# rostin79s/TFHE-AES

Measured on AMD Instinct MI355X. Metric: AES-128 CTR blocks/sec (FHE), higher is better.
Workload: dtype u64+f64; 1 GPU; configs[2]: 128 CTR blocks per GPU, Server::aes_encrypt 10 rounds (1280 bit-CBS/block), counters pre-incremented client-side; params=PARAM_OPT, blocks_per_gpu=128, total_blocks=128

## Files before the change

### tfhe_aes_amd/csrc/aes_schedule.h

```cpp
#pragma once

static int many_sbox_dev(fheaes_ctx *c, const uint64_t *bytes, uint64_t n_bytes, int set, uint64_t *out)
{
    return wopbs_dev(c, bytes, n_bytes, 8, c->lutset_d[set], (uint32_t)c->lutset_n[set], 0, out);
}

static int aes_rounds(uint32_t key_bits) { return key_bits == 128 ? 10 : key_bits == 192 ? 12 : key_bits == 256 ? 14 : 0; }

static int check_key_bits(fheaes_ctx *c, uint32_t key_bits)
{
    if (!aes_rounds(key_bits)) return c->fail(FHEAES_ERR_INVALID, "key_bits must be 128, 192 or 256, got %u", key_bits);
    return FHEAES_OK;
}

struct AesStep { int set; uint32_t n_luts; GatherTable table; int key_round; };
struct AesSchedule {
    int first_key_round = 0;
    uint32_t max_luts = 0;
    std::vector<AesStep> steps;
    void add(int set, uint32_t n_luts, const GatherTable &t, int key_round) { steps.push_back({set, n_luts, t, key_round}); max_luts = std::max(max_luts, n_luts); }
};

static AesSchedule aes_encrypt_schedule(int nr)
{
    AesSchedule s;
    s.first_key_round = 0;
    for (int round = 1; round < nr; ++round) s.add(LUTSET_ENC_ROUND, 3, table_enc_round(), round);
    s.add(LUTSET_SBOX, 1, table_shift_rows(false), nr);
    return s;
}

static AesSchedule aes_decrypt_schedule(int nr)
{
    AesSchedule s;
    s.first_key_round = nr;
    for (int round = nr; round >= 2; --round) {
        s.add(LUTSET_INV_SBOX, 1, table_shift_rows(true), round - 1);
        s.add(LUTSET_DEC_MUL, 4, table_dec_mix(), -1);
    }
    s.add(LUTSET_INV_SBOX, 1, table_shift_rows(true), 0);
    return s;
}

static AesSchedule aes_decrypt_eq_schedule(int nr)
{
    AesSchedule s;
    s.first_key_round = nr;
    for (int round = nr - 1; round >= 1; --round) s.add(LUTSET_DEC_EQ_ROUND, 4, table_dec_eq_round(), round);
    s.add(LUTSET_INV_SBOX, 1, table_shift_rows(true), 0);
    return s;
}

static int aes_run_dev(fheaes_ctx *c, const KeySets &rk, uint64_t *state, uint64_t n_blocks, const AesSchedule &sch)
{
    const uint64_t bw = 8ull * c->big1, sw = 16 * bw, steps = sch.steps.size();
    auto key_of = [&](const AesStep &st, uint64_t first_block) {
        if (st.key_round < 0) return KeySets{nullptr, nullptr, 0};
        return rk.round((uint64_t)st.key_round, sw, first_block);
    };
    const uint64_t w = aes_context_window(c, n_blocks, steps);
    TRY(ensure(c, c->ws_vp, (w ? w : n_blocks) * 16 * sch.max_luts * bw * 8));
    uint64_t *vp = (uint64_t *)c->ws_vp.p;
    TRY(launch_add_bcast(c, state, rk.round((uint64_t)sch.first_key_round, sw), sw, n_blocks));
    if (w == 0) {
        for (const AesStep &st : sch.steps) {
            TRY(many_sbox_dev(c, state, 16 * n_blocks, st.set, vp));
            TRY(launch_gather(c, vp, st.n_luts, key_of(st, 0), state, n_blocks, st.table));
        }
        return FHEAES_OK;
    }
    const uint64_t ggsw_words = (uint64_t)c->k1 * c->k1 * FHE_N, total = steps * n_blocks;
    TRY(ensure_wopbs_ws(c, w * AES_BLOCK_BITS));
    uint64_t *small = (uint64_t *)c->ws_small.p;
    const double2 *ggswf = (const double2 *)c->ws_ggswf.p;
    struct Segment { const AesStep *st; uint64_t first, blocks, row; uint64_t *vp; };
    for (uint64_t i0 = 0; i0 < total; i0 += w) {
        const uint64_t len = std::min<uint64_t>(w, total - i0), s = i0 / n_blocks, b0 = i0 % n_blocks, m = len * AES_BLOCK_BITS;
        Segment seg[2] = {{&sch.steps[s], b0, std::min<uint64_t>(len, n_blocks - b0), 0, vp}, {}};
        int n_seg = 1;
        if (seg[0].blocks < len) {
            seg[1] = {&sch.steps[s + 1], 0, len - seg[0].blocks, seg[0].blocks, vp + seg[0].blocks * 16 * seg[0].st->n_luts * bw};
            n_seg = 2;
        }
        for (int g = 0; g < n_seg; ++g)
            TRY(launch_keyswitch(c, state + seg[g].first * sw, seg[g].blocks * AES_BLOCK_BITS, small + seg[g].row * AES_BLOCK_BITS * (c->n + 1)));
        TRY(cbs_from_small(c, m));
        if (n_seg == 1 || seg[0].st->set == seg[1].st->set) {
            const int set = seg[0].st->set;
            TRY(launch_vertical_packing(c, ggswf, 16 * len, 8, c->lutset_d[set], (uint32_t)c->lutset_n[set], 0, vp));
        } else {
            for (int g = 0; g < n_seg; ++g) {
                const int set = seg[g].st->set;
                TRY(launch_vertical_packing(c, ggswf + seg[g].row * AES_BLOCK_BITS * (ggsw_words / 2), 16 * seg[g].blocks, 8, c->lutset_d[set],
                                            (uint32_t)c->lutset_n[set], 0, seg[g].vp));
            }
        }
        for (int g = 0; g < n_seg; ++g)
            TRY(launch_gather(c, seg[g].vp, seg[g].st->n_luts, key_of(*seg[g].st, seg[g].first), state + seg[g].first * sw, seg[g].blocks, seg[g].st->table));
    }
    return FHEAES_OK;
}

static int aes_encrypt_dev(fheaes_ctx *c, const KeySets &rk, uint64_t *state, uint64_t n_blocks, int nr) { return aes_run_dev(c, rk, state, n_blocks, aes_encrypt_schedule(nr)); }
static int aes_decrypt_dev(fheaes_ctx *c, const KeySets &rk, uint64_t *state, uint64_t n_blocks, int nr) { return aes_run_dev(c, rk, state, n_blocks, aes_decrypt_schedule(nr)); }
static int aes_decrypt_eq_dev(fheaes_ctx *c, const KeySets &dw, uint64_t *state, uint64_t n_blocks, int nr) { return aes_run_dev(c, dw, state, n_blocks, aes_decrypt_eq_schedule(nr)); }

typedef int (*AesDevFn)(fheaes_ctx *, const KeySets &, uint64_t *, uint64_t, int);

static int dec_round_keys_dev(fheaes_ctx *c, const uint64_t *w, uint64_t *dw, int nr, uint64_t n_keys)
{
    const uint64_t bw = 8ull * c->big1, sw = 16 * bw, ks = (uint64_t)(nr + 1) * sw, mid = (uint64_t)(nr - 1) * 16, nbytes = mid * n_keys;
    const bool strided = n_keys > 1;
    TRY(ensure(c, c->ws_vp, nbytes * 4 * bw * 8));
    TRY(ensure(c, c->ws_tmp_a, nbytes * bw * 8));
    if (strided) TRY(ensure(c, c->ws_tmp_b, nbytes * bw * 8));
    uint64_t *vp = (uint64_t *)c->ws_vp.p, *mix = (uint64_t *)c->ws_tmp_a.p, *flat = (uint64_t *)c->ws_tmp_b.p;
    TRY(launch_key_rows(c, dw, ks, w, ks, 0, nullptr, 0, 0, 16, n_keys, 1));
    TRY(launch_key_rows(c, dw + (uint64_t)nr * sw, ks, w + (uint64_t)nr * sw, ks, 0, nullptr, 0, 0, 16, n_keys, 1));
    if (strided) TRY(launch_key_rows(c, flat, mid * bw, w + sw, ks, 0, nullptr, 0, 0, (uint32_t)mid, n_keys, 1));
    TRY(many_sbox_dev(c, strided ? flat : w + sw, nbytes, LUTSET_DEC_MUL, vp));
    TRY(launch_gather(c, vp, 4, KeySets{nullptr, nullptr, 0}, mix, nbytes / 16, table_dec_mix()));
    TRY(many_sbox_dev(c, mix, nbytes, LUTSET_IDENTITY, strided ? flat : dw + sw));
    if (strided) TRY(launch_key_rows(c, dw + sw, ks, flat, mid * bw, 0, nullptr, 0, 0, (uint32_t)mid, n_keys, 1));
    return FHEAES_OK;
}

static int key_expansion_dev(fheaes_ctx *c, const uint64_t *key, uint64_t *w, int nr, uint64_t n_keys)
{
    static const uint8_t RCON[10] = {0x01, 0x02, 0x04, 0x08, 0x10, 0x20, 0x40, 0x80, 0x1B, 0x36};
    const uint64_t bw = 8ull * c->big1, ww = 4 * bw, ks = (uint64_t)(nr + 1) * 16 * bw;
    const int nk = nr - 6;
    const bool strided = n_keys > 1;
    TRY(ensure(c, c->ws_tmp_a, n_keys * ww * 8));
    TRY(ensure(c, c->ws_tmp_b, n_keys * ww * 8));
    if (strided) TRY(ensure(c, c->ws_tmp_c, n_keys * ww * 8));
    uint64_t *ta = (uint64_t *)c->ws_tmp_a.p, *tb = (uint64_t *)c->ws_tmp_b.p, *tc = (uint64_t *)c->ws_tmp_c.p;
    TRY(launch_key_rows(c, w, ks, key, (uint64_t)nk * ww, 0, nullptr, 0, 0, 4u * nk, n_keys, 1));
    for (int i = nk; i < 4 * (nr + 1); ++i) {
        const uint64_t *prev = w + (uint64_t)(i - 1) * ww, *back = w + (uint64_t)(i - nk) * ww;
        if (i % nk == 0) {
            TRY(launch_key_rows(c, ta, ww, prev, ks, 1, nullptr, 0, 0, 4, n_keys, 1));
            TRY(many_sbox_dev(c, ta, 4 * n_keys, LUTSET_SBOX, tb));
            TRY(launch_key_rows(c, ta, ww, tb, ww, 0, back, ks, RCON[i / nk - 1], 4, n_keys, 2));
        } else if (nk > 6 && i % nk == 4) {
            if (strided) TRY(launch_key_rows(c, ta, ww, prev, ks, 0, nullptr, 0, 0, 4, n_keys, 1));
            TRY(many_sbox_dev(c, strided ? ta : prev, 4 * n_keys, LUTSET_SBOX, tb));
            TRY(launch_key_rows(c, ta, ww, tb, ww, 0, back, ks, 0, 4, n_keys, 2));
        } else {
            TRY(launch_key_rows(c, ta, ww, prev, ks, 0, back, ks, 0, 4, n_keys, 2));
        }
        uint64_t *fresh = w + (uint64_t)i * ww;
        TRY(many_sbox_dev(c, ta, 4 * n_keys, LUTSET_IDENTITY, strided ? tc : fresh));
        if (strided) TRY(launch_key_rows(c, fresh, ks, tc, ww, 0, nullptr, 0, 0, 4, n_keys, 1));
    }
    return FHEAES_OK;
}

template <class Fill> static int upload_pinned(fheaes_ctx *c, size_t bytes, size_t ws_bytes, Fill fill)
{
    if (c->pin_ev) HIP_TRY(c, hipEventSynchronize(c->pin_ev));
    else HIP_TRY(c, hipEventCreateWithFlags(&c->pin_ev, hipEventDisableTiming));
    if (c->pin_bytes < bytes) {
        if (c->pin) { HIP_TRY(c, hipHostFree(c->pin)); c->pin = nullptr; c->pin_bytes = 0; }
        HIP_TRY(c, hipHostMalloc((void **)&c->pin, bytes, hipHostMallocDefault));
        c->pin_bytes = bytes;
    }
    fill(c->pin);
    TRY(ensure(c, c->ws_misc, ws_bytes));
    HIP_TRY(c, hipMemcpyAsync(c->ws_misc.p, c->pin, bytes, hipMemcpyHostToDevice, c->stream));
// ... 440 lines not shown
```

### tfhe_aes_amd/csrc/engine.hip

```cpp
#include <hip/hip_runtime.h>
#include <algorithm>
#include <cmath>
#include <cstdarg>
#include <cstdio>
#include <atomic>
#include <chrono>
#include <cstring>
#include <functional>
#include <mutex>
#include <string>
#include <type_traits>
#include <unordered_map>
#include <vector>

#include "knobs.h"
#include "fheaes.h"
#include "fft_dev.h"
#include "kern_extprod.h"
#include "kern_gate.h"
#include "kern_blindrot_latency.h"
#include "kern_blindrot16.h"
#include "kern_blindrot_pair.h"
#include "kern_audit.h"
#include "ks_launch.h"
// ... 1652 lines not shown
    Staged st(c, memspace);
    TRY(k.stage(st));
    TRY(st.out(keys_out, out_bytes, &keys_out));
    TRY(st.out(valid_out, valid_bytes, &valid_out));
    const bool table = k.n_keys > 1;
    const size_t tab_bytes = table ? (n_keys * sizeof(uint32_t) + 31) / 32 * 32 : 0, data_bytes = n_keys * 8 * (semiblocks + 1);
    TRY(upload_pinned(c, tab_bytes + data_bytes, tab_bytes + data_bytes, [&](uint8_t *pin) {
        if (table) memcpy(pin, k.key_of, n_keys * sizeof(uint32_t));
        memcpy(pin + tab_bytes, wrapped, data_bytes);
    }));
    const uint8_t *misc = (const uint8_t *)c->ws_misc.p;
    TRY(kw_unwrap_dev(c, k.sets(table ? (const uint32_t *)misc : nullptr), k.nr, misc + tab_bytes, semiblocks, n_keys, keys_out, valid_out));
    return st.finish();
}

int fheaes_aes_kw_unwrap_keyed(fheaes_ctx *c, const uint64_t *dec_round_keys, uint32_t key_bits, uint64_t n_keks, uint64_t n_keys, const uint32_t *kek_of_key,
                               uint32_t semiblocks, const uint8_t *wrapped, uint64_t *keys_out, uint64_t *valid_out, int memspace)
{
    return aes_kw_unwrap(c, {dec_round_keys, key_bits, n_keks, kek_of_key, n_keys, false}, semiblocks, wrapped, keys_out, valid_out, memspace);
}

int fheaes_aes_kw_unwrap_keyed_packed(fheaes_ctx *c, const uint64_t *packed_dec_round_keys, uint32_t key_bits, uint64_t n_keks, uint64_t n_keys,
                                      const uint32_t *kek_of_key, uint32_t semiblocks, const uint8_t *wrapped, uint64_t *keys_out, uint64_t *valid_out, int memspace)
{
    return aes_kw_unwrap(c, {packed_dec_round_keys, key_bits, n_keks, kek_of_key, n_keys, true}, semiblocks, wrapped, keys_out, valid_out, memspace);
}

int fheaes_aes_kw_plan(uint32_t key_bits, uint32_t semiblocks, uint64_t n_keys, uint64_t *steps, uint64_t *cipher_blocks, uint64_t *byte_wopbs)
{
    const uint64_t nr = (uint64_t)aes_rounds(key_bits), n = semiblocks;
    if (!nr || n < KW_MIN_SEMIBLOCKS || n > KW_MAX_SEMIBLOCKS || n_keys > FHEAES_KW_MAX_KEYS || !steps || !cipher_blocks || !byte_wopbs) return FHEAES_ERR_INVALID;
    *steps = 6 * n;
    *cipher_blocks = 6 * n * n_keys;
    *byte_wopbs = 16 * nr * 6 * n * n_keys + 8 * n * n_keys + 16 * n_keys;
    return FHEAES_OK;
}

static_assert(GATE_LWE == FHEAES_GATE_LWE && GATE_GLWE == FHEAES_GATE_GLWE, "fheaes.h's input forms are the kernel's");

static int gate_call(fheaes_ctx *c, bool boot, const double *ggsw_fourier, const uint64_t *gates_lwe, uint64_t n_gates, const uint64_t *bits_of_gate, const uint64_t *in,
                     uint64_t m, int form, uint64_t *out, int memspace)
{
    if (!c) return FHEAES_ERR_INVALID;
    CtxLock lock__(c);
    if (boot) TRY(check_keys(c));
    if (form != GATE_LWE && form != GATE_GLWE) return c->fail(FHEAES_ERR_INVALID, "form must be 0 (LWE) or 1 (GLWE), got %d", form);
    if (n_gates && !bits_of_gate) return c->fail(FHEAES_ERR_INVALID, "null pointer");
    if (n_gates > 0xFFFFFFFFull) return c->fail(FHEAES_ERR_INVALID, "a call takes at most 2^32 - 1 gates (got %llu)", (unsigned long long)n_gates);
    const uint32_t R = gate_r(c->k1);
    const uint64_t chunk = boot ? MAX_CHUNK_BITS : 0;
    std::vector<GateWg> wgs;
    std::vector<uint64_t> chunk_end;
    uint64_t n_wgs = 0, total = 0;
    for (uint64_t g = 0; g < n_gates; ++g) {
        if (bits_of_gate[g] > m - total) { total = ~0ull; break; }
        total += bits_of_gate[g];
    }
    if (total != m) return c->fail(FHEAES_ERR_INVALID, "the runs of bits_of_gate do not add up to m = %llu", (unsigned long long)m);
    if (m == 0) return FHEAES_OK;
    if (!in || !out || (boot ? !gates_lwe : !ggsw_fourier)) return c->fail(FHEAES_ERR_INVALID, "null pointer");
    const uint64_t ggsw_words = (uint64_t)c->k1 * c->k1 * FHE_N, inst_words = form == GATE_GLWE ? (uint64_t)c->k1 * FHE_N : c->big1;
    const uint64_t bytes = m * inst_words * 8, gate_bytes = n_gates * (boot ? c->big1 : ggsw_words) * 8;
    const void *gates = boot ? (const void *)gates_lwe : (const void *)ggsw_fourier;
    if (out != in && overlap(in, bytes, out, bytes)) return c->fail(FHEAES_ERR_INVALID, "in and out overlap without being the same buffer");
    if (overlap(gates, gate_bytes, out, bytes)) return c->fail(FHEAES_ERR_INVALID, "out overlaps the gates");
    gate_table(bits_of_gate, n_gates, R, chunk, &wgs, &chunk_end, &n_wgs);
    HIP_TRY(c, hipSetDevice(c->device));
    Staged s(c, memspace);
    if (boot) TRY(s.in(gates_lwe, gate_bytes, &gates_lwe));
    else TRY(s.in(ggsw_fourier, gate_bytes, &ggsw_fourier));
    if (out == in) { TRY(s.inout(out, bytes, &out)); in = out; }
    else { TRY(s.in(in, bytes, &in)); TRY(s.out(out, bytes, &out)); }
    const size_t tab_bytes = wgs.size() * sizeof(GateWg);
    TRY(upload_pinned(c, tab_bytes, tab_bytes, [&](uint8_t *pin) { memcpy(pin, wgs.data(), tab_bytes); }));
    const GateWg *tab = (const GateWg *)c->ws_misc.p;
    if (!boot) {
        TRY(launch_gate(c, (const double2 *)ggsw_fourier, tab, n_wgs, m, form, in, out));
        return s.finish();
    }
    TRY(ensure_wopbs_ws(c, std::min<uint64_t>(n_gates, chunk)));
    uint64_t wg0 = 0;
    for (uint64_t g0 = 0, ci = 0; g0 < n_gates; g0 += chunk, ++ci) {
        const uint64_t gc = std::min<uint64_t>(chunk, n_gates - g0);
        TRY(cbs_bits(c, gates_lwe + g0 * c->big1, gc));
        uint64_t units = 0;
        for (uint64_t g = g0; g < g0 + gc; ++g) units += bits_of_gate[g];
        TRY(launch_gate(c, (const double2 *)c->ws_ggswf.p, tab + wg0, chunk_end[ci] - wg0, units, form, in, out));
        wg0 = chunk_end[ci];
    }
    return s.finish();
}

int fheaes_gate_ggsw(fheaes_ctx *c, const double *ggsw_fourier, uint64_t n_gates, const uint64_t *bits_of_gate, const uint64_t *in, uint64_t m, int form,
                     uint64_t *out, int memspace)
{
    return gate_call(c, false, ggsw_fourier, nullptr, n_gates, bits_of_gate, in, m, form, out, memspace);
}

int fheaes_gate_bits(fheaes_ctx *c, const uint64_t *gates_lwe, uint64_t n_gates, const uint64_t *bits_of_gate, const uint64_t *lwe_in, uint64_t m,
                     uint64_t *lwe_out, int memspace)
{
    return gate_call(c, true, nullptr, gates_lwe, n_gates, bits_of_gate, lwe_in, m, GATE_LWE, lwe_out, memspace);
}

int fheaes_gate_packed(fheaes_ctx *c, const uint64_t *gates_lwe, uint64_t n_gates, const uint64_t *glwes_of_gate, const uint64_t *glwe_in, uint64_t n_glwe,
                       uint64_t *glwe_out, int memspace)
{
    return gate_call(c, true, nullptr, gates_lwe, n_gates, glwes_of_gate, glwe_in, n_glwe, GATE_GLWE, glwe_out, memspace);
}

int fheaes_gate_plan(const uint64_t *bits_of_gate, uint64_t n_gates, uint32_t k, uint64_t *workgroups, uint32_t *instances_per_workgroup)
{
    if ((n_gates && !bits_of_gate) || (k != 4 && k != 1) || !workgroups || !instances_per_workgroup) return FHEAES_ERR_INVALID;
    *instances_per_workgroup = gate_r(k + 1);
    gate_table(bits_of_gate, n_gates, *instances_per_workgroup, 0, nullptr, nullptr, workgroups);
    return FHEAES_OK;
}

size_t fheaes_packed_words(const fheaes_ctx *c, uint64_t m)
{
    if (!c) return 0;
    return (size_t)((m + FHE_N - 1) / FHE_N) * c->k1 * FHE_N;
}

int fheaes_pack_bits(fheaes_ctx *c, const uint64_t *lwe_in, uint64_t m, uint64_t *glwe_out, int memspace)
{
    if (!c) return FHEAES_ERR_INVALID;
    CtxLock lock__(c);
    TRY(check_keys(c));
    if (m == 0) return FHEAES_OK;
    if (!lwe_in || !glwe_out) return c->fail(FHEAES_ERR_INVALID, "null pointer");
    const uint64_t in_bytes = m * c->big1 * 8, out_bytes = (uint64_t)fheaes_packed_words(c, m) * 8;
    if (overlap(lwe_in, in_bytes, glwe_out, out_bytes)) return c->fail(FHEAES_ERR_INVALID, "lwe_in and glwe_out overlap (packing is not in place)");
    HIP_TRY(c, hipSetDevice(c->device));
    Staged s(c, memspace);
    TRY(s.in(lwe_in, in_bytes, &lwe_in));
    TRY(s.out(glwe_out, out_bytes, &glwe_out));
    TRY(pack_dev(c, lwe_in, m, glwe_out));
    return s.finish();
}

int fheaes_unpack_bits(fheaes_ctx *c, const uint64_t *glwe_in, uint64_t m, uint64_t *lwe_out, int memspace)
{
    if (!c) return FHEAES_ERR_INVALID;
    CtxLock lock__(c);
    if (m == 0) return FHEAES_OK;
    if (!glwe_in || !lwe_out) return c->fail(FHEAES_ERR_INVALID, "null pointer");
    const uint64_t in_bytes = (uint64_t)fheaes_packed_words(c, m) * 8, out_bytes = m * c->big1 * 8;
    if (overlap(glwe_in, in_bytes, lwe_out, out_bytes)) return c->fail(FHEAES_ERR_INVALID, "glwe_in and lwe_out overlap (unpacking is not in place)");
    HIP_TRY(c, hipSetDevice(c->device));
    Staged s(c, memspace);
    TRY(s.in(glwe_in, in_bytes, &glwe_in));
    TRY(s.out(lwe_out, out_bytes, &lwe_out));
    TRY(unpack_dev(c, glwe_in, m, lwe_out));
    return s.finish();
}

uint32_t fheaes_round_keys_packed_glwes(uint32_t key_bits) { return packed_key_glwes(key_bits); }

int fheaes_pack_round_keys(fheaes_ctx *c, const uint64_t *round_keys, uint32_t key_bits, uint64_t n_keys, uint64_t *packed_out, int memspace)
{
    CtxLock lock__(c);
    TRY(check_keys(c));
    if (!round_keys || !packed_out) return c->fail(FHEAES_ERR_INVALID, "null pointer");
    TRY(check_key_bits(c, key_bits));
    TRY(check_n_keys(c, n_keys));
    const uint64_t m = (uint64_t)(aes_rounds(key_bits) + 1) * AES_BLOCK_BITS, glwes = packed_key_glwes(key_bits);
// ... 152 lines not shown
```

### tfhe_aes_amd/csrc/engine_launch.h

```cpp
#pragma once

#define MAX_CHUNK_BITS 32768ull
#define K2_CALL_MAX_BITS 65536ull
#define MAX_WOPBS_BITS 16u

namespace {

#define LATENCY_BATCH_BITS 256ull
#define K2_PAIR_MIN_BITS 768ull
struct K2Plan { int form; uint64_t units_main; uint32_t r_main; uint64_t units_tail; uint32_t r_tail; };
K2Plan k2_plan(uint64_t m, uint32_t cu_count, uint32_t k1, bool allow_pair = true)
{
    K2Plan pl{};
    if (m <= LATENCY_BATCH_BITS) { pl.form = 0; pl.units_main = m; pl.r_main = 1; return pl; }
    if (allow_pair && k1 == 5 && m > K2_PAIR_MIN_BITS) {
        pl.form = 2; pl.r_main = 6; pl.r_tail = 4;
        const uint64_t gens = (m + 6ull * cu_count - 1) / (6ull * cu_count);
        uint64_t nu = gens * cu_count;
        uint64_t four = 6 * nu >= m ? (6 * nu - m) / 2 : 0;
        if (four > nu) four = nu;
        if (four == nu && 4 * nu > m) { nu = (m + 3) / 4; four = nu; }
        pl.units_tail = four; pl.units_main = nu - four;
        return pl;
    }
    pl.form = 1;
    pl.r_main = k1 == 5 ? 3 : 8;
    pl.units_main = (m + pl.r_main - 1) / pl.r_main;
    if (k1 == 5) {
        const uint64_t slots = 2ull * cu_count;
        pl.r_tail = 2;
        if ((m + 1) / 2 <= cu_count) {
            pl.units_main = 0;
            pl.units_tail = (m + 1) / 2;
        } else if (pl.units_main > slots) {
            const uint64_t nu = slots * ((m + 3 * slots - 1) / (3 * slots));
            if (2 * nu <= m) {
                pl.units_tail = 3 * nu - m;
                pl.units_main = nu - pl.units_tail;
            }
        }
    }
    return pl;
}

#define AES_BLOCK_BITS 128ull
#define AES_WINDOW_MAX_BLOCKS (MAX_CHUNK_BITS / AES_BLOCK_BITS)
struct AesWindowPlan { uint64_t window, launches, generations, generations_by_round; };

uint64_t k2_generations(uint64_t m, uint32_t cu_count, uint32_t k1)
{
    if (m == 0) return 0;
    if (m <= K2_PAIR_MIN_BITS) return 1;
    const K2Plan pl = k2_plan(m, cu_count, k1);
    return (pl.units_main + pl.units_tail + cu_count - 1) / cu_count;
}

void aes_window_count(uint64_t n, uint64_t steps, uint64_t w, uint32_t cu_count, uint32_t k1, uint64_t *launches, uint64_t *generations)
{
    const uint64_t total = steps * n, full = total / w, rest = total % w;
    *launches = full + (rest ? 1 : 0);
    *generations = full * k2_generations(w * AES_BLOCK_BITS, cu_count, k1) + k2_generations(rest * AES_BLOCK_BITS, cu_count, k1);
}

AesWindowPlan aes_window_plan(uint64_t n, uint64_t steps, uint32_t cu_count, uint32_t k1, bool allow_pair = true)
{
    AesWindowPlan pl{};
    const uint64_t chunks = n / AES_WINDOW_MAX_BLOCKS, last = n % AES_WINDOW_MAX_BLOCKS;
    pl.launches = steps * (chunks + (last ? 1 : 0));
    pl.generations_by_round = steps * (chunks * k2_generations(MAX_CHUNK_BITS, cu_count, k1) + k2_generations(last * AES_BLOCK_BITS, cu_count, k1));
    pl.generations = pl.generations_by_round;
    if (n == 0 || steps == 0) return pl;
    const uint64_t gen_bits = 6ull * cu_count;
    if (k2_plan(std::min<uint64_t>(n * AES_BLOCK_BITS, MAX_CHUNK_BITS), cu_count, k1, allow_pair).form != 2) return pl;
    if (n * AES_BLOCK_BITS % gen_bits == 0) return pl;
    uint64_t g = AES_BLOCK_BITS, r = gen_bits;
    while (r) { const uint64_t t = g % r; g = r; r = t; }
    const uint64_t base = gen_bits / g;
    const uint64_t w = std::min<uint64_t>(n, AES_WINDOW_MAX_BLOCKS) / base * base;
    if (w == 0) return pl;
    uint64_t launches, generations;
    aes_window_count(n, steps, w, cu_count, k1, &launches, &generations);
    if (generations >= pl.generations_by_round) return pl;
    pl.window = w; pl.launches = launches; pl.generations = generations;
    return pl;
}

int launch_keyswitch(fheaes_ctx *c, const uint64_t *in, uint64_t m, uint64_t *out)
{
    if (m == 0) return FHEAES_OK;
    StageScope sc(c, FHEAES_STAGE_KEYSWITCH, m);
    const uint64_t ct_tiles16 = ((m + KS_CT_TILE - 1) / KS_CT_TILE) * (KS_CT_TILE / 16);
    TRY(ensure(c, c->ws_digits, ct_tiles16 * c->ks_ksteps * 1024));
    int8_t *af = (int8_t *)c->ws_digits.p;
    const uint64_t threads = ct_tiles16 * c->ks_ksteps * 64;
    ks_launch_digits_k1(dim3((unsigned)((threads + 255) / 256)), c->stream, in, (uint64_t)c->big1, c->big, m, c->ks_ksteps, af);
    KeyswitchArgs a{};
    a.afrag = af; a.bfrag = c->ksk_frag; a.ksteps = c->ks_ksteps; a.coltiles = c->ks_coltiles;
    a.in = in; a.in_stride = c->big1; a.body_index = (int32_t)c->big; a.body_col = c->n; a.ncols = c->n + 1;
    a.out = out; a.out_stride = c->n + 1; a.out_z_stride = 0; a.m = m;
    dim3 grid((c->ks_coltiles + KSL_COL_TILES - 1) / KSL_COL_TILES, (unsigned)((m + 16 * KSL_CT_TILES - 1) / (16 * KSL_CT_TILES)), 1);
    ks_launch_mfma_lds(1, grid, c->stream, a);
    HIP_TRY(c, hipGetLastError());
    return FHEAES_OK;
}

int launch_pfpks(fheaes_ctx *c, const uint64_t *in, uint64_t m, uint64_t *out, uint64_t out_stride, int block = -1)
{
    if (m == 0) return FHEAES_OK;
    StageScope sc(c, FHEAES_STAGE_PFPKS, m);
    const uint32_t gsz = c->k1 * FHE_N;
    const uint64_t ct_tiles16 = ((m + KS_CT_TILE - 1) / KS_CT_TILE) * (KS_CT_TILE / 16);
    TRY(ensure(c, c->ws_digits, ct_tiles16 * c->pf_ksteps * 2 * 1024));
    int8_t *af = (int8_t *)c->ws_digits.p;
    const uint64_t threads = ct_tiles16 * c->pf_ksteps * 64;
    ks_launch_digits_k3(dim3((unsigned)((threads + 255) / 256)), c->stream, in, (uint64_t)c->big1, c->big1, m, c->pf_ksteps, af);
    KeyswitchArgs a{};
    a.afrag = af; a.bfrag = c->pfpksk_frag; a.ksteps = c->pf_ksteps; a.coltiles = c->pf_coltiles;
    if (block >= 0) a.bfrag += (size_t)block * c->pf_ksteps * c->pf_coltiles * 8 * 1024;
    a.in = in; a.in_stride = c->big1; a.body_index = -1; a.body_col = 0; a.ncols = gsz;
    a.out = out; a.out_stride = out_stride; a.out_z_stride = block >= 0 ? 0 : gsz; a.m = m;
    dim3 grid((c->pf_coltiles + KSL_COL_TILES - 1) / KSL_COL_TILES, (unsigned)((m + 16 * KSL_CT_TILES - 1) / (16 * KSL_CT_TILES)), block >= 0 ? 1 : c->k1);
    ks_launch_mfma_lds(2, grid, c->stream, a);
    HIP_TRY(c, hipGetLastError());
    return FHEAES_OK;
}

int launch_forward_fourier(fheaes_ctx *c, const uint64_t *in, uint64_t polys, double2 *out, int stage)
{
    if (polys == 0) return FHEAES_OK;
    StageScope sc(c, stage, polys);
    uint64_t wgs = (polys + EP_GROUPS - 1) / EP_GROUPS;
    if (wgs > 8192) wgs = 8192;
    hipLaunchKernelGGL(forward_fourier_kernel, dim3((unsigned)wgs), dim3(EP_THREADS), 0, c->stream, in, out, polys, c->tw_d);
    HIP_TRY(c, hipGetLastError());
    return FHEAES_OK;
}

bool k2_pair_allowed(fheaes_ctx *c)
{
    if (c->k2_deny_pair) return false;
    if (c->k2_pair_ok < 0) {
        int per_cu = 0;
        const hipError_t oe = hipOccupancyMaxActiveBlocksPerMultiprocessor(&per_cu, blind_rotate_pair_kernel<5, 5, 8, 3, 2>, BRP_THREADS, 0);
        c->k2_pair_ok = (oe == hipSuccess && per_cu >= 1) ? 1 : 0;
        (void)hipGetLastError();
    }
    return c->k2_pair_ok == 1;
}

bool k2_home_allowed(fheaes_ctx *c)
{
    if (c->k1 != 5 || c->k2_deny_home) return false;
    if (c->k2_home < 0) {
        int per_cu = 0;
        const hipError_t oe = hipOccupancyMaxActiveBlocksPerMultiprocessor(&per_cu, blind_rotate16_kernel<5, 5, 8, 3, 2, true>, EP_THREADS, 0);
        c->k2_home = (oe == hipSuccess && per_cu >= 2) ? 1 : 0;
        (void)hipGetLastError();
    }
    return c->k2_home == 1;
}

static_assert(FHEAES_K2_PARK_SLOTS == BRP_PARK_SLOTS, "include/fheaes.h and kern_blindrot_pair.h disagree on the number of parking slots");
constexpr size_t PARK_OWNER_BYTES = BRP_PARK_SLOTS * sizeof(uint32_t) + BRP_PARK_TAIL_WORDS * sizeof(uint64_t);
constexpr size_t PARK_RECORD_PTR_OFFSET = BRP_PARK_SLOTS * sizeof(uint32_t) + 2 * sizeof(uint64_t);

int ensure_park_owner(fheaes_ctx *c)
{
    if (c->ws_park_owner.p) return FHEAES_OK;
    TRY(ensure(c, c->ws_park_owner, PARK_OWNER_BYTES));
    HIP_TRY(c, hipMemsetAsync(c->ws_park_owner.p, 0, PARK_OWNER_BYTES, c->stream));
    return FHEAES_OK;
}

size_t k2_pair_park_bytes(const fheaes_ctx *c, uint64_t grid)
{
    return (size_t)((c->k2_park_claim ? BRP_PARK_SLOTS : 0) + grid) * 2 * BRP_PARK_WORDS_PER_HALF * 8;
}

struct K2Launch {
    K2Plan pl;
    void (*kernel)(ExtProdArgs);
    const char *name;
    unsigned grid, threads;
    size_t park_bytes;
    bool park_owner;
};
K2Launch k2_launch(fheaes_ctx *c, uint64_t m)
{
    K2Launch L{};
    L.pl = k2_plan(m, c->cu_count, c->k1, k2_pair_allowed(c));
    L.grid = (unsigned)(L.pl.units_main + L.pl.units_tail);
    if (L.pl.form == 0) {
        L.threads = BL_THREADS;
        if (c->k1 == 5) { L.kernel = blind_rotate_latency_kernel<5, 5, 8>; L.name = "blind_rotate_latency_kernel<5,5,8>"; }
        else { L.kernel = blind_rotate_latency_kernel<2, 5, 8>; L.name = "blind_rotate_latency_kernel<2,5,8>"; }
    } else if (L.pl.form == 2) {
        L.threads = BRP_THREADS;
        L.kernel = blind_rotate_pair_kernel<5, 5, 8, 3, 2>;
        L.name = c->k2_park_claim ? "blind_rotate_pair_kernel<5,5,8,3,2> parking=claimed" : "blind_rotate_pair_kernel<5,5,8,3,2> parking=private";
        L.park_bytes = k2_pair_park_bytes(c, L.grid);
        L.park_owner = c->k2_park_claim != 0;
    } else {
        L.threads = EP_THREADS;
// ... 356 lines not shown
{
    const uint64_t gsz = (uint64_t)c->k1 * FHE_N, glwes = (m + FHE_N - 1) / FHE_N, max_keys = MAX_CHUNK_BITS / m;
    uint64_t chunk = c->ws_ggsw.bytes / (gsz * 8) / m;
    if (chunk == 0) {
        chunk = std::min<uint64_t>(n_keys, max_keys);
        TRY(ensure(c, c->ws_ggsw, chunk * m * gsz * 8));
    }
    chunk = std::min<uint64_t>(chunk, max_keys);
    uint64_t *ks = (uint64_t *)c->ws_ggsw.p;
    for (uint64_t j0 = 0; j0 < n_keys; j0 += chunk) {
        const uint64_t kc = std::min<uint64_t>(chunk, n_keys - j0);
        TRY(launch_pfpks(c, in + j0 * m * c->big1, kc * m, ks, gsz, (int)c->k));
        uint64_t *o = out + j0 * glwes * gsz;
        StageScope sc(c, FHEAES_STAGE_LINEAR, kc * m);
        HIP_TRY(c, hipMemsetAsync(o, 0, kc * glwes * gsz * 8, c->stream));
        for (uint64_t j = 0; j < kc; ++j)
            hipLaunchKernelGGL(pack_fold_kernel, dim3(FHE_N / PACK_FOLD_ROWS, c->k1, (unsigned)glwes), dim3(256), 0, c->stream, ks + j * m * gsz, m, c->k1,
                               o + j * glwes * gsz);
        HIP_TRY(c, hipGetLastError());
    }
    return FHEAES_OK;
}

int unpack_keys_dev(fheaes_ctx *c, const uint64_t *in, uint64_t m, uint64_t n_keys, uint64_t *out)
{
    const uint64_t key_words = (m + FHE_N - 1) / FHE_N * c->k1 * FHE_N;
    for (uint64_t j = 0; j < n_keys; ++j) TRY(unpack_dev(c, in + j * key_words, m, out + j * m * c->big1));
    return FHEAES_OK;
}

int mod_switch_dev(fheaes_ctx *c, const uint64_t *in, uint64_t n_glwe, uint32_t width, uint64_t *out)
{
    const uint64_t gsz = (uint64_t)c->k1 * FHE_N, step = MAX_CHUNK_BITS / FHE_N;
    for (uint64_t g0 = 0; g0 < n_glwe; g0 += step) {
        const uint64_t gc = std::min<uint64_t>(step, n_glwe - g0);
        StageScope sc(c, FHEAES_STAGE_LINEAR, gc * FHE_N);
        launch_mod_switch(c, in + g0 * gsz, gc, width, out + g0 * (gsz / 64 * width));
        HIP_TRY(c, hipGetLastError());
    }
    return FHEAES_OK;
}

int unpack_mod_dev(fheaes_ctx *c, const uint64_t *in, uint64_t m, uint32_t width, uint64_t *out)
{
    for (uint64_t t0 = 0; t0 < m; t0 += MAX_CHUNK_BITS) {
        const uint64_t mc = std::min<uint64_t>(MAX_CHUNK_BITS, m - t0);
        StageScope sc(c, FHEAES_STAGE_LINEAR, mc);
        hipLaunchKernelGGL(sample_extract_mod_kernel, dim3((unsigned)((mc + UNPACK_BITS_PER_WG - 1) / UNPACK_BITS_PER_WG)), dim3(256), 0, c->stream,
                           in + t0 / FHE_N * (uint64_t)c->k1 * 8 * width, mc, c->k, width, out + t0 * c->big1);
        HIP_TRY(c, hipGetLastError());
    }
    return FHEAES_OK;
}

int expand_lwe_dev(fheaes_ctx *c, const MaskKey &key, uint64_t first_index, const uint64_t *bodies, uint64_t m, uint64_t *out)
{
    for (uint64_t t0 = 0; t0 < m; t0 += MAX_CHUNK_BITS) {
        const uint64_t mc = std::min<uint64_t>(MAX_CHUNK_BITS, m - t0);
        StageScope sc(c, FHEAES_STAGE_LINEAR, mc);
        hipLaunchKernelGGL(expand_lwe_kernel, dim3((unsigned)((mc * c->k + 3) / 4)), dim3(256), 0, c->stream, out + t0 * c->big1, bodies + t0, mc, c->k,
                           first_index + t0, key);
        HIP_TRY(c, hipGetLastError());
    }
    return FHEAES_OK;
}

int check_keys(fheaes_ctx *c)
{
    if (!c) return FHEAES_ERR_INVALID;
    if (!c->have_keys) return c->fail(FHEAES_ERR_NOKEYS, "evaluation keys have not been uploaded");
    return FHEAES_OK;
}

int ensure_wopbs_ws(fheaes_ctx *c, uint64_t bits)
{
    const uint64_t ggsw_words = (uint64_t)c->k1 * c->k1 * FHE_N;
    TRY(ensure(c, c->ws_small, bits * (c->n + 1) * 8));
    TRY(ensure(c, c->ws_pbs, bits * c->big1 * 8));
    TRY(ensure(c, c->ws_ggsw, bits * ggsw_words * 8));
    TRY(ensure(c, c->ws_ggswf, bits * ggsw_words * 8));
    return FHEAES_OK;
}

int cbs_from_small(fheaes_ctx *c, uint64_t m)
{
    const uint64_t ggsw_words = (uint64_t)c->k1 * c->k1 * FHE_N;
    TRY(launch_cbs_pbs(c, (const uint64_t *)c->ws_small.p, m, 1, (uint64_t *)c->ws_pbs.p));
    TRY(launch_pfpks(c, (const uint64_t *)c->ws_pbs.p, m, (uint64_t *)c->ws_ggsw.p, ggsw_words));
    TRY(launch_forward_fourier(c, (const uint64_t *)c->ws_ggsw.p, m * c->k1 * c->k1, (double2 *)c->ws_ggswf.p, FHEAES_STAGE_GGSW_FFT));
    return FHEAES_OK;
}

int cbs_bits(fheaes_ctx *c, const uint64_t *in, uint64_t m)
{
    TRY(launch_keyswitch(c, in, m, (uint64_t *)c->ws_small.p));
    return cbs_from_small(c, m);
}

int wopbs_dev(fheaes_ctx *c, const uint64_t *lwe_in, uint64_t n_inputs, uint32_t bits, const uint64_t *luts, uint32_t n_luts,
              int per_input, uint64_t *lwe_out)
{
    if (bits < 1 || bits > MAX_WOPBS_BITS) return c->fail(FHEAES_ERR_INVALID, "bits_per_input must be in 1..%u (got %u)", MAX_WOPBS_BITS, bits);
    if (n_luts < 1) return c->fail(FHEAES_ERR_INVALID, "n_luts must be >= 1");
    if (n_inputs == 0) return FHEAES_OK;
    uint64_t chunk_inputs = std::max<uint64_t>(1, MAX_CHUNK_BITS / bits);
    if (bits > 9) {
        const uint64_t per_input = (uint64_t)n_luts * bits * (1ull << (bits - 9)) * c->k1 * FHE_N * 8;
        chunk_inputs = std::max<uint64_t>(1, std::min<uint64_t>(chunk_inputs, (2ull << 30) / per_input));
    }
    const uint64_t W = lut_row_words(bits);
    TRY(ensure_wopbs_ws(c, std::min<uint64_t>(n_inputs, chunk_inputs) * bits));
    for (uint64_t i0 = 0; i0 < n_inputs; i0 += chunk_inputs) {
        const uint64_t ni = std::min<uint64_t>(chunk_inputs, n_inputs - i0);
        TRY(cbs_bits(c, lwe_in + i0 * bits * c->big1, ni * bits));
        const uint64_t *l = per_input ? luts + i0 * n_luts * bits * W : luts;
        TRY(launch_vertical_packing(c, (const double2 *)c->ws_ggswf.p, ni, bits, l, n_luts, per_input, lwe_out + i0 * n_luts * bits * c->big1));
    }
    return FHEAES_OK;
}

}
```

### tfhe_aes_amd/csrc/kern_keyswitch.h

```cpp
#pragma once
#include <hip/hip_runtime.h>
#include <stdint.h>
#include "fft_dev.h"

#define KS_CT_TILE 64
#define KS_KSTEP 64

typedef int ks_int4 __attribute__((ext_vector_type(4)));

struct KeyswitchArgs {
    const int8_t *afrag;
    const int8_t *bfrag;
    uint32_t ksteps, coltiles;
    const uint64_t *in;
    uint64_t in_stride;
    int32_t body_index;
    uint32_t body_col;
    uint32_t ncols;
    uint64_t *out;
    uint64_t out_stride, out_z_stride;
    uint64_t m;
};

#define KSL_CT_TILES 8
#define KSL_THREADS (64 * KSL_CT_TILES)
#define KSL_COL_TILES 4

#ifndef FHEAES_KS_DECLS_ONLY
__global__ __launch_bounds__(256) void keybytes_kernel(const uint64_t *key, uint64_t key_z_stride, uint32_t rows, uint32_t ncols,
                                                       uint32_t ksteps, uint32_t coltiles, int8_t *frag)
{
    const uint64_t gid = (uint64_t)blockIdx.x * blockDim.x + threadIdx.x;
    const uint32_t lane = gid & 63;
    const uint64_t t = gid >> 6;
    const uint32_t C = t % coltiles;
    const uint32_t ks = (uint32_t)(t / coltiles);
    const uint32_t z = blockIdx.y;
    if (ks >= ksteps) return;
    const uint32_t col = C * 16 + (lane & 15);
    const uint32_t row0 = ks * KS_KSTEP + (lane >> 4) * 16;
    int8_t b[8][16];
#pragma unroll
    for (int e = 0; e < 16; ++e) {
        uint64_t x = 0;
        if (col < ncols && row0 + e < rows) x = key[(uint64_t)z * key_z_stride + (uint64_t)(row0 + e) * ncols + col];
        uint32_t carry = 0;
#pragma unroll
        for (int j = 0; j < 8; ++j) {
            uint32_t v = (uint32_t)((x >> (8 * j)) & 0xFF) + carry;
            carry = v >= 128 ? 1u : 0u;
            b[j][e] = (int8_t)(v & 0xFF);
        }
    }
    int8_t *o = frag + ((((uint64_t)z * ksteps + ks) * coltiles + C) * 8) * 1024 + (uint64_t)lane * 16;
#pragma unroll
    for (int j = 0; j < 8; ++j) {
        ks_int4 w;
        memcpy(&w, b[j], 16);
        *reinterpret_cast<ks_int4 *>(o + (uint64_t)j * 1024) = w;
    }
}

template <int BASE_LOG, int LEVELS, int PLANES>
__global__ __launch_bounds__(256) void digits_kernel(const uint64_t *in, uint64_t in_stride, uint32_t n_in, uint64_t m,
                                                     uint32_t ksteps, int8_t *frag)
{
    const uint64_t gid = (uint64_t)blockIdx.x * blockDim.x + threadIdx.x;
    const uint32_t lane = gid & 63;
    const uint64_t t = gid >> 6;
    const uint32_t ks = t % ksteps;
    const uint64_t T = t / ksteps;
    const uint64_t ct = T * 16 + (lane & 15);
    const uint32_t q0 = ks * KS_KSTEP + (lane >> 4) * 16;
    int8_t lo[16], hi[16];
#pragma unroll
    for (int e = 0; e < 16; ++e) { lo[e] = 0; hi[e] = 0; }
    if (ct < m) {
        const uint32_t i0 = q0 / LEVELS;
        constexpr int NI = (16 + LEVELS - 1) / LEVELS + 1;
#pragma unroll
        for (int ii = 0; ii < NI; ++ii) {
            const uint32_t i = i0 + ii;
            if (i >= n_in) break;
            int d[LEVELS];
            decompose_all<BASE_LOG, LEVELS>(in[ct * in_stride + i], d);
#pragma unroll
            for (int l = 0; l < LEVELS; ++l) {
                const int e = (int)(i * LEVELS + l) - (int)q0;
                if (e >= 0 && e < 16) {
                    const int dl = ((d[l] + 128) & 255) - 128;
#pragma unroll
                    for (int ee = 0; ee < 16; ++ee) if (ee == e) { lo[ee] = (int8_t)dl; hi[ee] = (int8_t)((d[l] - dl) >> 8); }
                }
            }
        }
    }
    int8_t *o = frag + ((T * ksteps + ks) * PLANES) * 1024 + (uint64_t)lane * 16;
    ks_int4 w;
    memcpy(&w, lo, 16);
    *reinterpret_cast<ks_int4 *>(o) = w;
    if (PLANES == 2) {
        memcpy(&w, hi, 16);
        *reinterpret_cast<ks_int4 *>(o + 1024) = w;
    }
}

template <int PLANES>
__global__ __launch_bounds__(KSL_THREADS, 2) void keyswitch_mfma_lds_kernel(const KeyswitchArgs A)
{
    constexpr int A_FRAGS = KSL_CT_TILES * PLANES;
    constexpr int B_FRAGS = KSL_COL_TILES * 8;
    constexpr int FRAGS = A_FRAGS + B_FRAGS;
    __shared__ __attribute__((aligned(16))) int8_t lds[2 * FRAGS * 1024];
    const int lane = threadIdx.x & 63, wave = threadIdx.x >> 6;
    const int wc = wave & 3, wt = wave >> 2;
    const uint32_t C0 = blockIdx.x * KSL_COL_TILES;
    const uint64_t T0 = (uint64_t)blockIdx.y * KSL_CT_TILES;
    const uint32_t z = blockIdx.z;
    const uint64_t ct_tiles_total = (A.m + 15) / 16;

    ks_int4 acc[4][8];
#pragma unroll
    for (int t = 0; t < 4; ++t)
#pragma unroll
        for (int s = 0; s < 8; ++s) acc[t][s] = (ks_int4){0, 0, 0, 0};

    auto issue = [&](uint32_t ks, int buf) {
        constexpr int WAVES = KSL_THREADS / 64;
#pragma unroll
        for (int i = 0; i < (FRAGS + WAVES - 1) / WAVES; ++i) {
            const int f = wave + WAVES * i;
            if (f < FRAGS) {
                const int8_t *src;
                if (f < A_FRAGS) {
                    uint64_t T = T0 + f / PLANES;
                    if (T >= ct_tiles_total) T = ct_tiles_total - 1;
                    src = A.afrag + ((T * A.ksteps + ks) * PLANES + (f % PLANES)) * 1024;
                } else {
                    const int g = f - A_FRAGS;
                    uint32_t C = C0 + g / 8;
                    if (C >= A.coltiles) C = A.coltiles - 1;
                    src = A.bfrag + ((((uint64_t)z * A.ksteps + ks) * A.coltiles + C) * 8 + (g % 8)) * 1024;
                }
                __builtin_amdgcn_global_load_lds((const __attribute__((address_space(1))) void *)(src + lane * 16),
                                                 (__attribute__((address_space(3))) void *)(lds + ((size_t)buf * FRAGS + f) * 1024), 16, 0, 0);
            }
        }
    };

    issue(0, 0);
    for (uint32_t ks = 0; ks < A.ksteps; ++ks) {
        const int buf = ks & 1;
        asm volatile("s_waitcnt vmcnt(0)" ::: "memory");
        __syncthreads();
        if (ks + 1 < A.ksteps) issue(ks + 1, buf ^ 1);
        const int8_t *base = lds + (size_t)buf * FRAGS * 1024 + lane * 16;
        ks_int4 a[4][PLANES], b[8];
#pragma unroll
        for (int s = 0; s < 8; ++s) b[s] = *reinterpret_cast<const ks_int4 *>(base + (A_FRAGS + wc * 8 + s) * 1024);
#pragma unroll
        for (int t = 0; t < 4; ++t)
#pragma unroll
            for (int pl = 0; pl < PLANES; ++pl) a[t][pl] = *reinterpret_cast<const ks_int4 *>(base + ((wt * 4 + t) * PLANES + pl) * 1024);
#pragma unroll
        for (int s = 0; s < 8; ++s) {
#pragma unroll
            for (int t = 0; t < 4; ++t) acc[t][s] = __builtin_amdgcn_mfma_i32_16x16x64_i8(a[t][0], b[s], acc[t][s], 0, 0, 0);
            if (PLANES == 2 && s >= 1) {
#pragma unroll
                for (int t = 0; t < 4; ++t) acc[t][s] = __builtin_amdgcn_mfma_i32_16x16x64_i8(a[t][1], b[s - 1], acc[t][s], 0, 0, 0);
            }
        }
    }

    const uint32_t C = C0 + wc;
    const uint32_t col = C * 16 + (lane & 15);
    if (C >= A.coltiles || col >= A.ncols) return;
#pragma unroll
    for (int t = 0; t < 4; ++t)
#pragma unroll
        for (int r = 0; r < 4; ++r) {
            const uint64_t ct = (T0 + wt * 4 + t) * 16 + (uint64_t)(lane >> 4) * 4 + r;
            if (ct >= A.m) continue;
            uint64_t v = 0;
#pragma unroll
            for (int s = 0; s < 8; ++s) v += (uint64_t)(int64_t)acc[t][s][r] << (8 * s);
            v = (uint64_t)0 - v;
            if (A.body_index >= 0 && col == A.body_col) v += A.in[ct * A.in_stride + (uint32_t)A.body_index];
            A.out[ct * A.out_stride + (uint64_t)z * A.out_z_stride + col] = v;
        }
}
#endif
```

### tfhe_aes_amd/csrc/ks_launch.h

```cpp
#pragma once
#ifdef FHEAES_SPLIT_KS
#ifndef FHEAES_KS_TU
#define FHEAES_KS_DECLS_ONLY
#endif
#endif
#include "kern_keyswitch.h"

#if defined(FHEAES_SPLIT_KS) && !defined(FHEAES_KS_TU)
#define FHEAES_KS_LAUNCH_DECL
#else
#define FHEAES_KS_LAUNCH_DEFINE
#ifdef FHEAES_SPLIT_KS
#define FHEAES_KS_LAUNCH_LINKAGE
#else
#define FHEAES_KS_LAUNCH_LINKAGE static inline
#endif
#endif

#ifdef FHEAES_KS_LAUNCH_DECL
void ks_launch_digits_k1(dim3 grid, hipStream_t s, const uint64_t *in, uint64_t in_stride, uint32_t n_in, uint64_t m, uint32_t ksteps, int8_t *frag);
void ks_launch_digits_k3(dim3 grid, hipStream_t s, const uint64_t *in, uint64_t in_stride, uint32_t n_in, uint64_t m, uint32_t ksteps, int8_t *frag);
void ks_launch_mfma_lds(int planes, dim3 grid, hipStream_t s, const KeyswitchArgs &a);
void ks_launch_keybytes(dim3 grid, hipStream_t s, const uint64_t *key, uint64_t key_z_stride, uint32_t rows, uint32_t ncols, uint32_t ksteps,
                        uint32_t coltiles, int8_t *frag);
#endif

#ifdef FHEAES_KS_LAUNCH_DEFINE
FHEAES_KS_LAUNCH_LINKAGE void ks_launch_digits_k1(dim3 grid, hipStream_t s, const uint64_t *in, uint64_t in_stride, uint32_t n_in, uint64_t m, uint32_t ksteps, int8_t *frag)
{
    hipLaunchKernelGGL((digits_kernel<2, 6, 1>), grid, dim3(256), 0, s, in, in_stride, n_in, m, ksteps, frag);
}
FHEAES_KS_LAUNCH_LINKAGE void ks_launch_digits_k3(dim3 grid, hipStream_t s, const uint64_t *in, uint64_t in_stride, uint32_t n_in, uint64_t m, uint32_t ksteps, int8_t *frag)
{
    hipLaunchKernelGGL((digits_kernel<12, 3, 2>), grid, dim3(256), 0, s, in, in_stride, n_in, m, ksteps, frag);
}
FHEAES_KS_LAUNCH_LINKAGE void ks_launch_mfma_lds(int planes, dim3 grid, hipStream_t s, const KeyswitchArgs &a)
{
    if (planes == 1) hipLaunchKernelGGL((keyswitch_mfma_lds_kernel<1>), grid, dim3(KSL_THREADS), 0, s, a);
    else hipLaunchKernelGGL((keyswitch_mfma_lds_kernel<2>), grid, dim3(KSL_THREADS), 0, s, a);
}
FHEAES_KS_LAUNCH_LINKAGE void ks_launch_keybytes(dim3 grid, hipStream_t s, const uint64_t *key, uint64_t key_z_stride, uint32_t rows, uint32_t ncols, uint32_t ksteps,
                                          uint32_t coltiles, int8_t *frag)
{
    hipLaunchKernelGGL(keybytes_kernel, grid, dim3(256), 0, s, key, key_z_stride, rows, ncols, ksteps, coltiles, frag);
}
#endif
```

Baseline: 58.52 blocks/s.

## Skip unused PFPKS mask outputs for bit-0 of 8-bit LUT inputs

Adds a row permutation in the private functional packing keyswitch so that bit 0 of each 8-bit vertical-packing input lands in dedicated 16-row tiles. The MFMA keyswitch kernel then skips those tiles for all GGSW rows except the last, on the assumption that vertical packing only needs the body row for the least significant bit. This cuts keyswitch work during AES S-box circuit bootstrapping. It relies on the mapping assumptions holding (m a multiple of 1024, downstream never reading the skipped rows) and adds index arithmetic to the digits and output paths.

```diff
diff --git a/tfhe_aes_amd/csrc/aes_schedule.h b/tfhe_aes_amd/csrc/aes_schedule.h
--- a/tfhe_aes_amd/csrc/aes_schedule.h
+++ b/tfhe_aes_amd/csrc/aes_schedule.h
@@ -84,7 +84,7 @@
         }
         for (int g = 0; g < n_seg; ++g)
             TRY(launch_keyswitch(c, state + seg[g].first * sw, seg[g].blocks * AES_BLOCK_BITS, small + seg[g].row * AES_BLOCK_BITS * (c->n + 1)));
-        TRY(cbs_from_small(c, m));
+        TRY(cbs_from_small(c, m, 8));
         if (n_seg == 1 || seg[0].st->set == seg[1].st->set) {
             const int set = seg[0].st->set;
             TRY(launch_vertical_packing(c, ggswf, 16 * len, 8, c->lutset_d[set], (uint32_t)c->lutset_n[set], 0, vp));
diff --git a/tfhe_aes_amd/csrc/engine.hip b/tfhe_aes_amd/csrc/engine.hip
--- a/tfhe_aes_amd/csrc/engine.hip
+++ b/tfhe_aes_amd/csrc/engine.hip
@@ -1758,7 +1758,7 @@
     uint64_t wg0 = 0;
     for (uint64_t g0 = 0, ci = 0; g0 < n_gates; g0 += chunk, ++ci) {
         const uint64_t gc = std::min<uint64_t>(chunk, n_gates - g0);
-        TRY(cbs_bits(c, gates_lwe + g0 * c->big1, gc));
+        TRY(cbs_bits(c, gates_lwe + g0 * c->big1, gc, 0));
         uint64_t units = 0;
         for (uint64_t g = g0; g < g0 + gc; ++g) units += bits_of_gate[g];
         TRY(launch_gate(c, (const double2 *)c->ws_ggswf.p, tab + wg0, chunk_end[ci] - wg0, units, form, in, out));
diff --git a/tfhe_aes_amd/csrc/engine_launch.h b/tfhe_aes_amd/csrc/engine_launch.h
--- a/tfhe_aes_amd/csrc/engine_launch.h
+++ b/tfhe_aes_amd/csrc/engine_launch.h
@@ -104,21 +104,22 @@
     return FHEAES_OK;
 }
 
-int launch_pfpks(fheaes_ctx *c, const uint64_t *in, uint64_t m, uint64_t *out, uint64_t out_stride, int block = -1)
+int launch_pfpks(fheaes_ctx *c, const uint64_t *in, uint64_t m, uint64_t *out, uint64_t out_stride, int block = -1, uint32_t lut_bits = 0)
 {
     if (m == 0) return FHEAES_OK;
     StageScope sc(c, FHEAES_STAGE_PFPKS, m);
     const uint32_t gsz = c->k1 * FHE_N;
+    const uint32_t row_map = (lut_bits == 8 && block < 0 && m % KS_MAP_BLOCK == 0) ? 8u : 0u;
     const uint64_t ct_tiles16 = ((m + KS_CT_TILE - 1) / KS_CT_TILE) * (KS_CT_TILE / 16);
     TRY(ensure(c, c->ws_digits, ct_tiles16 * c->pf_ksteps * 2 * 1024));
     int8_t *af = (int8_t *)c->ws_digits.p;
     const uint64_t threads = ct_tiles16 * c->pf_ksteps * 64;
-    ks_launch_digits_k3(dim3((unsigned)((threads + 255) / 256)), c->stream, in, (uint64_t)c->big1, c->big1, m, c->pf_ksteps, af);
+    ks_launch_digits_k3(dim3((unsigned)((threads + 255) / 256)), c->stream, in, (uint64_t)c->big1, c->big1, m, c->pf_ksteps, af, row_map);
     KeyswitchArgs a{};
     a.afrag = af; a.bfrag = c->pfpksk_frag; a.ksteps = c->pf_ksteps; a.coltiles = c->pf_coltiles;
     if (block >= 0) a.bfrag += (size_t)block * c->pf_ksteps * c->pf_coltiles * 8 * 1024;
     a.in = in; a.in_stride = c->big1; a.body_index = -1; a.body_col = 0; a.ncols = gsz;
-    a.out = out; a.out_stride = out_stride; a.out_z_stride = block >= 0 ? 0 : gsz; a.m = m;
+    a.out = out; a.out_stride = out_stride; a.out_z_stride = block >= 0 ? 0 : gsz; a.m = m; a.row_map = row_map;
     dim3 grid((c->pf_coltiles + KSL_COL_TILES - 1) / KSL_COL_TILES, (unsigned)((m + 16 * KSL_CT_TILES - 1) / (16 * KSL_CT_TILES)), block >= 0 ? 1 : c->k1);
     ks_launch_mfma_lds(2, grid, c->stream, a);
     HIP_TRY(c, hipGetLastError());
@@ -641,19 +642,19 @@
     return FHEAES_OK;
 }
 
-int cbs_from_small(fheaes_ctx *c, uint64_t m)
+int cbs_from_small(fheaes_ctx *c, uint64_t m, uint32_t lut_bits)
 {
     const uint64_t ggsw_words = (uint64_t)c->k1 * c->k1 * FHE_N;
     TRY(launch_cbs_pbs(c, (const uint64_t *)c->ws_small.p, m, 1, (uint64_t *)c->ws_pbs.p));
-    TRY(launch_pfpks(c, (const uint64_t *)c->ws_pbs.p, m, (uint64_t *)c->ws_ggsw.p, ggsw_words));
+    TRY(launch_pfpks(c, (const uint64_t *)c->ws_pbs.p, m, (uint64_t *)c->ws_ggsw.p, ggsw_words, -1, lut_bits));
     TRY(launch_forward_fourier(c, (const uint64_t *)c->ws_ggsw.p, m * c->k1 * c->k1, (double2 *)c->ws_ggswf.p, FHEAES_STAGE_GGSW_FFT));
     return FHEAES_OK;
 }
 
-int cbs_bits(fheaes_ctx *c, const uint64_t *in, uint64_t m)
+int cbs_bits(fheaes_ctx *c, const uint64_t *in, uint64_t m, uint32_t lut_bits)
 {
     TRY(launch_keyswitch(c, in, m, (uint64_t *)c->ws_small.p));
-    return cbs_from_small(c, m);
+    return cbs_from_small(c, m, lut_bits);
 }
 
 int wopbs_dev(fheaes_ctx *c, const uint64_t *lwe_in, uint64_t n_inputs, uint32_t bits, const uint64_t *luts, uint32_t n_luts,
@@ -671,7 +672,7 @@
     TRY(ensure_wopbs_ws(c, std::min<uint64_t>(n_inputs, chunk_inputs) * bits));
     for (uint64_t i0 = 0; i0 < n_inputs; i0 += chunk_inputs) {
         const uint64_t ni = std::min<uint64_t>(chunk_inputs, n_inputs - i0);
-        TRY(cbs_bits(c, lwe_in + i0 * bits * c->big1, ni * bits));
+        TRY(cbs_bits(c, lwe_in + i0 * bits * c->big1, ni * bits, bits == 8 ? 8u : 0u));
         const uint64_t *l = per_input ? luts + i0 * n_luts * bits * W : luts;
         TRY(launch_vertical_packing(c, (const double2 *)c->ws_ggswf.p, ni, bits, l, n_luts, per_input, lwe_out + i0 * n_luts * bits * c->big1));
     }
diff --git a/tfhe_aes_amd/csrc/kern_keyswitch.h b/tfhe_aes_amd/csrc/kern_keyswitch.h
--- a/tfhe_aes_amd/csrc/kern_keyswitch.h
+++ b/tfhe_aes_amd/csrc/kern_keyswitch.h
@@ -20,7 +20,29 @@
     uint64_t *out;
     uint64_t out_stride, out_z_stride;
     uint64_t m;
+    uint32_t row_map;
 };
+
+#define KS_MAP_BLOCK 1024u
+#define KS_MAP_REST 896u
+#if defined(__HIPCC__) || defined(__CUDACC__)
+#define KS_HD __host__ __device__
+#else
+#define KS_HD
+#endif
+KS_HD static inline uint64_t ks_row_to_ct(uint64_t row)
+{
+    const uint32_t r = (uint32_t)(row % KS_MAP_BLOCK);
+    const uint32_t j = r < KS_MAP_REST ? r + r / 7 + 1 : (r - KS_MAP_REST) * 8;
+    return row - r + j;
+}
+KS_HD static inline uint64_t ks_ct_to_row(uint64_t ct)
+{
+    const uint32_t j = (uint32_t)(ct % KS_MAP_BLOCK);
+    const uint32_t r = j % 8 ? j - j / 8 - 1 : KS_MAP_REST + j / 8;
+    return ct - j + r;
+}
+KS_HD static inline bool ks_tile_is_bit0(uint64_t tile) { return tile % 8 == 7; }
 
 #define KSL_CT_TILES 8
 #define KSL_THREADS (64 * KSL_CT_TILES)
@@ -63,14 +85,15 @@
 
 template <int BASE_LOG, int LEVELS, int PLANES>
 __global__ __launch_bounds__(256) void digits_kernel(const uint64_t *in, uint64_t in_stride, uint32_t n_in, uint64_t m,
-                                                     uint32_t ksteps, int8_t *frag)
+                                                     uint32_t ksteps, int8_t *frag, uint32_t row_map)
 {
     const uint64_t gid = (uint64_t)blockIdx.x * blockDim.x + threadIdx.x;
     const uint32_t lane = gid & 63;
     const uint64_t t = gid >> 6;
     const uint32_t ks = t % ksteps;
     const uint64_t T = t / ksteps;
-    const uint64_t ct = T * 16 + (lane & 15);
+    const uint64_t row = T * 16 + (lane & 15);
+    const uint64_t ct = row_map ? ks_row_to_ct(row) : row;
     const uint32_t q0 = ks * KS_KSTEP + (lane >> 4) * 16;
     int8_t lo[16], hi[16];
 #pragma unroll
@@ -118,6 +141,7 @@
     const uint64_t T0 = (uint64_t)blockIdx.y * KSL_CT_TILES;
     const uint32_t z = blockIdx.z;
     const uint64_t ct_tiles_total = (A.m + 15) / 16;
+    if (A.row_map && z + 1 < gridDim.z && ks_tile_is_bit0(blockIdx.y)) return;
 
     ks_int4 acc[4][8];
 #pragma unroll
@@ -180,7 +204,8 @@
     for (int t = 0; t < 4; ++t)
 #pragma unroll
         for (int r = 0; r < 4; ++r) {
-            const uint64_t ct = (T0 + wt * 4 + t) * 16 + (uint64_t)(lane >> 4) * 4 + r;
+            const uint64_t row = (T0 + wt * 4 + t) * 16 + (uint64_t)(lane >> 4) * 4 + r;
+            const uint64_t ct = A.row_map ? ks_row_to_ct(row) : row;
             if (ct >= A.m) continue;
             uint64_t v = 0;
 #pragma unroll
diff --git a/tfhe_aes_amd/csrc/ks_launch.h b/tfhe_aes_amd/csrc/ks_launch.h
--- a/tfhe_aes_amd/csrc/ks_launch.h
+++ b/tfhe_aes_amd/csrc/ks_launch.h
@@ -19,7 +19,8 @@
 
 #ifdef FHEAES_KS_LAUNCH_DECL
 void ks_launch_digits_k1(dim3 grid, hipStream_t s, const uint64_t *in, uint64_t in_stride, uint32_t n_in, uint64_t m, uint32_t ksteps, int8_t *frag);
-void ks_launch_digits_k3(dim3 grid, hipStream_t s, const uint64_t *in, uint64_t in_stride, uint32_t n_in, uint64_t m, uint32_t ksteps, int8_t *frag);
+void ks_launch_digits_k3(dim3 grid, hipStream_t s, const uint64_t *in, uint64_t in_stride, uint32_t n_in, uint64_t m, uint32_t ksteps, int8_t *frag,
+                         uint32_t row_map);
 void ks_launch_mfma_lds(int planes, dim3 grid, hipStream_t s, const KeyswitchArgs &a);
 void ks_launch_keybytes(dim3 grid, hipStream_t s, const uint64_t *key, uint64_t key_z_stride, uint32_t rows, uint32_t ncols, uint32_t ksteps,
                         uint32_t coltiles, int8_t *frag);
@@ -28,11 +29,12 @@
 #ifdef FHEAES_KS_LAUNCH_DEFINE
 FHEAES_KS_LAUNCH_LINKAGE void ks_launch_digits_k1(dim3 grid, hipStream_t s, const uint64_t *in, uint64_t in_stride, uint32_t n_in, uint64_t m, uint32_t ksteps, int8_t *frag)
 {
-    hipLaunchKernelGGL((digits_kernel<2, 6, 1>), grid, dim3(256), 0, s, in, in_stride, n_in, m, ksteps, frag);
+    hipLaunchKernelGGL((digits_kernel<2, 6, 1>), grid, dim3(256), 0, s, in, in_stride, n_in, m, ksteps, frag, 0u);
 }
-FHEAES_KS_LAUNCH_LINKAGE void ks_launch_digits_k3(dim3 grid, hipStream_t s, const uint64_t *in, uint64_t in_stride, uint32_t n_in, uint64_t m, uint32_t ksteps, int8_t *frag)
+FHEAES_KS_LAUNCH_LINKAGE void ks_launch_digits_k3(dim3 grid, hipStream_t s, const uint64_t *in, uint64_t in_stride, uint32_t n_in, uint64_t m, uint32_t ksteps, int8_t *frag,
+                                           uint32_t row_map)
 {
-    hipLaunchKernelGGL((digits_kernel<12, 3, 2>), grid, dim3(256), 0, s, in, in_stride, n_in, m, ksteps, frag);
+    hipLaunchKernelGGL((digits_kernel<12, 3, 2>), grid, dim3(256), 0, s, in, in_stride, n_in, m, ksteps, frag, row_map);
 }
 FHEAES_KS_LAUNCH_LINKAGE void ks_launch_mfma_lds(int planes, dim3 grid, hipStream_t s, const KeyswitchArgs &a)
 {
```

Result: no change. 58.84 blocks/s (median of 6 runs) (+0.5%).
